# dbolya/yolact

Measured on AMD Instinct MI355X. Metric: images/sec (550x550, batch 8 per GPU), YOLACT yolact_resnet50 forward + Detect (Fast NMS), higher is better.
Workload: dtype f32 (fp32 in / fp32 accumulate / fp32 out; 93 % of the GEMM time on fp16x2 tiles = every fp32 operand as two fp16 pieces by round to nearest (22 significant bits + 2 signs: exact for ~2/3 of all fp32 values, one fp32 ulp otherwise), 3 exact piece products per product on the fp16 matrix pipe; measure

## Files before the change

include/yolact_amd.h:

```cpp
#ifndef YOLACT_AMD_H
#define YOLACT_AMD_H
#include <stddef.h>
#include <stdint.h>

#ifdef __cplusplus
extern "C" {
#endif

#define YMI_ABI_VERSION 9

#define YMI_EFORMAT (-4)
#define YMI_EUNSUPPORTED (-5)

enum { YMI_ACT_NONE = 0, YMI_ACT_RELU = 1, YMI_ACT_LEAKY01 = 2, YMI_ACT_TANH = 3, YMI_ACT_SIGMOID = 4 };
enum { YMI_RES_NONE = 0, YMI_RES_ADD = 1, YMI_RES_BILINEAR = 2 };

typedef struct {
  int32_t n0, n1;
  int32_t act;
  int32_t row_stride;
  int64_t batch_stride;
  float *ptr;
} ymi_conv_seg;

// ... 217 lines not shown
  int32_t out_width, out_height;
  int32_t hs[3], vs[3];
  int32_t hf[3], vf[3];
  int32_t bw[3], bh[3];
  int32_t dw[3], dh[3];
  int64_t coef_count;
  int64_t plane_bytes;
} ymi_jpeg_info;
int ymi_jpeg_parse(const uint8_t *data, size_t n, ymi_jpeg_info *info);
int ymi_jpeg_decode_coefs(const uint8_t *data, size_t n, int16_t *coefs, int64_t coef_capacity, uint16_t *qt,
                          ymi_jpeg_info *info);
int ymi_jpeg_reconstruct_bgr_u8(const ymi_jpeg_info *info, const int16_t *coefs, const uint16_t *qt, uint8_t *planes_ws,
                                uint8_t *out, void *stream);

int ymi_coco_poly_fill_u8(const double *xy, int k, int h, int w, uint8_t *mask);
int ymi_coco_rle_fill_u8(const uint32_t *counts, long n, int h, int w, uint8_t *mask);
int ymi_coco_rle_string_fill_u8(const char *s, long len, int h, int w, uint8_t *mask);

typedef struct {
  ymi_conv_desc conv;
  const float *offmask;
  int32_t ldo;
  int32_t mask_is_prob;
  int32_t om_layout;
  int32_t _pad1;
} ymi_dcn_desc;
int ymi_dcn_v2_forward_f32(const ymi_dcn_desc *d, void *stream);

typedef struct ymi_stem_desc {
  const float *x;
  float *y;
  int32_t B, H, W, cout_pad;
  const void *w_h2;
  const float *scale_h2, *bias;
  float *y_amax;
  int32_t kpad, _pad0;
} ymi_stem_desc;
int ymi_stem_pool_f32(const ymi_stem_desc *d, void *stream);

typedef struct ymi_chain_desc {
  const float *x, *res;
  float *y, *z;
  const void *w_a_h2, *w_b_h2;
  const float *scale_a_h2, *bias_a, *scale_b_h2, *bias_b;
  const float *x_amax;
  float *y_amax, *z_amax;
  int64_t M;
  int32_t ldx, res_ld, ldy, ldz;
  int32_t k_a, n_a, n_b;
  int32_t cout_pad_a, cout_pad_b;
  int32_t act_a, act_b, _pad0;
  const float *res_amax;
  float gain_a, bias_max_a;
} ymi_chain_desc;
int ymi_pointwise_chain_f32(const ymi_chain_desc *d, void *stream);

enum { YMI_OP_NOP = 0, YMI_OP_CONV = 1, YMI_OP_WINO = 2, YMI_OP_DCN = 3, YMI_OP_CHAIN = 4, YMI_OP_STEM = 5, YMI_OP_INPUT = 6,
       YMI_OP_BILINEAR = 7, YMI_OP_MAXPOOL = 8, YMI_OP_BILINEAR_ADD = 9, YMI_OP_RECORD = 10, YMI_OP_WAIT = 11, YMI_OP_MEMSET = 12 };
enum { YMI_SEC_NONE = 0, YMI_SEC_BACKBONE = 1, YMI_SEC_FPN = 2, YMI_SEC_PROTO = 3, YMI_SEC_HEADS = 4 };
typedef struct ymi_plan_op {
  int32_t kind;
  int32_t stream;
  int32_t section;
  int32_t _pad;
  const void *desc;
  void *p[3];
  int64_t i[8];
  double f[2];
} ymi_plan_op;
int ymi_event_create(void **ev);
int ymi_event_destroy(void *ev);
int ymi_plan_run(const ymi_plan_op *ops, int first, int last, void *stream_a, void *stream_b, void *const *events, int overlap,
                 int skip_sections, int32_t *failed_op);

enum {
  YMI_WS_WINO_V = 1,
  YMI_WS_WINO_M = 2,
  YMI_WS_SPLITK = 3,
  YMI_WS_MASK_IOU = 4,
  YMI_WS_JPEG_COEFS = 5,
  YMI_WS_JPEG_PLANES = 6,
  YMI_WS_DETECT_SCORES_T = 7,
  YMI_WS_DETECT_PER_PRIOR = 8,
  YMI_WS_DETECT_CAND = 9,
  YMI_WS_DETECT_REC = 10,
  YMI_WS_AMAX_SLOT = 11,
  YMI_WS_RLE_COUNTS = 12,
  YMI_WS_DETECT_GREEDY = 13
};
typedef struct { int32_t A, B; int64_t n; } ymi_mask_iou_shape;
typedef struct { int32_t N, h, w, cap; } ymi_rle_shape;
int64_t ymi_workspace_bytes(int what, const void *desc);

int ymi_calib_mfma_f16(float *out, int blocks, int iters, double *flops, void *stream);
int ymi_calib_hbm_copy(const float *src, float *dst, long n_floats, double *bytes, void *stream);
int ymi_calib_l2_read(const float *src, long n_floats, int blocks, int iters, float *out, double *bytes, void *stream);
int ymi_calib_latency(const int32_t *chain, long n, int start, int hops, int32_t *out, void *stream);

int ymi_debug_set_trace(void *buf, long cap_blocks);
int ymi_prof_enable(int on);
int ymi_prof_count(void);
int ymi_prof_read(int i, float *ms, double *flops, int32_t *tile, int32_t *kind);
int ymi_prof_reset(void);

#ifdef __cplusplus
}
// ... 3 lines not shown
```

yolact_amd/_lib.py:

```python
from __future__ import annotations

import ctypes as C
import os

_HERE = os.path.dirname(os.path.abspath(__file__))
LIB_PATH = os.path.join(_HERE, 'libyolact_amd.so')

ABI_VERSION = 9

ACT_NONE, ACT_RELU, ACT_LEAKY01, ACT_TANH, ACT_SIGMOID = 0, 1, 2, 3, 4
RES_NONE, RES_ADD, RES_BILINEAR = 0, 1, 2
TILE_AUTO, TILE_128x128, TILE_128x64, TILE_64x64, TILE_128x32, TILE_64x128 = 0, 1, 2, 3, 4, 5
TILE_32x32_K4, TILE_64x32_K2, TILE_32x64_K2 = 6, 7, 8
TILE_64x64_S3, TILE_64x64_S4, TILE_64x128_S3, TILE_128x64_S3, TILE_32x32_K4_S4, TILE_64x32_K2_S3, TILE_32x64_K2_S3 = range(9, 16)
TILE_NAMES = {1: '128x128', 2: '128x64', 3: '64x64', 4: '128x32', 5: '64x128', 6: '32x32k4', 7: '64x32k2', 8: '32x64k2',
              9: '64x64s3', 10: '64x64s4', 11: '64x128s3', 12: '128x64s3', 13: '32x32k4s4', 14: '64x32k2s3', 15: '32x64k2s3',
              16: '128x128w8', 17: '256x128w8', 18: '128x256w8', 19: '128x128s3', 20: '128x128w8s3', 21: '256x128w8s3',
              22: '128x128w8s4'}
TILE_128x128_W8, TILE_256x128_W8, TILE_128x256_W8 = 16, 17, 18
TILE_128x128_S3, TILE_128x128_W8_S3, TILE_256x128_W8_S3, TILE_128x128_W8_S4 = 19, 20, 21, 22
TILE_WG_128x256 = 23
TILE_X3 = 32
X3_BASE_TILES = (1, 2, 3, 5, 6, 7, 8, 9, 11, 12, 16, 17, 19, 20, 21, 22)
for _t in X3_BASE_TILES:
# ... 50 lines not shown


class WinoDesc(C.Structure):
    _fields_ = [('x', C.c_void_p), ('u', C.c_void_p), ('scale', C.c_void_p), ('bias', C.c_void_p), ('y', C.c_void_p),
                ('V', C.c_void_p), ('M', C.c_void_p),
                ('B', C.c_int32), ('H', C.c_int32), ('W', C.c_int32), ('C', C.c_int32), ('Cout', C.c_int32),
                ('act', C.c_int32), ('tile', C.c_int32), ('nseg', C.c_int32), ('m', C.c_int32), ('_pad0', C.c_int32),
                ('seg', ConvSeg * 3), ('u_x3', C.c_void_p), ('cout_alg', C.c_int32), ('v_planes', C.c_int32),
                ('u_h2', C.c_void_p), ('uinv_h2', C.c_void_p), ('x_amax', C.c_void_p), ('y_amax', C.c_void_p),
                ('x_up', C.c_void_p), ('up_relu', C.c_int32), ('_pad4', C.c_int32),
                ('proj_w_h2', C.c_void_p), ('proj_scale_h2', C.c_void_p), ('proj_bias', C.c_void_p),
                ('proj_y', C.c_void_p), ('proj_y_amax', C.c_void_p),
                ('proj_cout', C.c_int32), ('proj_ldy', C.c_int32), ('proj_act', C.c_int32), ('_pad5', C.c_int32)]


class DcnDesc(C.Structure):
    _fields_ = [('conv', ConvDesc), ('offmask', C.c_void_p), ('ldo', C.c_int32), ('mask_is_prob', C.c_int32),
                ('om_layout', C.c_int32), ('_pad1', C.c_int32)]


class DetectDesc(C.Structure):
    _fields_ = [('conf', C.c_void_p), ('loc', C.c_void_p), ('coef', C.c_void_p), ('priors', C.c_void_p),
                ('B', C.c_int32), ('P', C.c_int32), ('C', C.c_int32), ('D', C.c_int32),
                ('conf_is_logits', C.c_int32), ('top_k', C.c_int32), ('max_det', C.c_int32),
                ('conf_thresh', C.c_float), ('nms_thresh', C.c_float), ('cross_class', C.c_int32),
                ('conf_ld', C.c_int32), ('_pad1', C.c_int32),
                ('scores_t', C.c_void_p), ('keep', C.c_void_p), ('num_keep', C.c_void_p),
                ('maxsc', C.c_void_p), ('argmax', C.c_void_p),
                ('cand_score', C.c_void_p), ('cand_prior', C.c_void_p),
                ('out_count', C.c_void_p), ('out_box', C.c_void_p), ('out_score', C.c_void_p),
                ('out_class', C.c_void_p), ('out_coef', C.c_void_p), ('out_prior', C.c_void_p), ('out_rec', C.c_void_p)]


class DetectGreedyWs(C.Structure):
    _fields_ = [('box_scale', C.c_float), ('_pad0', C.c_int32), ('ws', C.c_void_p)]


class JpegInfo(C.Structure):
    _fields_ = [('width', C.c_int32), ('height', C.c_int32), ('ncomp', C.c_int32), ('progressive', C.c_int32),
                ('orientation', C.c_int32), ('color', C.c_int32), ('out_width', C.c_int32), ('out_height', C.c_int32),
                ('hs', C.c_int32 * 3), ('vs', C.c_int32 * 3), ('hf', C.c_int32 * 3), ('vf', C.c_int32 * 3),
                ('bw', C.c_int32 * 3), ('bh', C.c_int32 * 3), ('dw', C.c_int32 * 3), ('dh', C.c_int32 * 3),
                ('coef_count', C.c_int64), ('plane_bytes', C.c_int64)]


class ChainDesc(C.Structure):
    _fields_ = [('x', C.c_void_p), ('res', C.c_void_p), ('y', C.c_void_p), ('z', C.c_void_p),
                ('w_a_h2', C.c_void_p), ('w_b_h2', C.c_void_p),
                ('scale_a_h2', C.c_void_p), ('bias_a', C.c_void_p), ('scale_b_h2', C.c_void_p), ('bias_b', C.c_void_p),
                ('x_amax', C.c_void_p), ('y_amax', C.c_void_p), ('z_amax', C.c_void_p),
                ('M', C.c_int64), ('ldx', C.c_int32), ('res_ld', C.c_int32), ('ldy', C.c_int32), ('ldz', C.c_int32),
                ('k_a', C.c_int32), ('n_a', C.c_int32), ('n_b', C.c_int32), ('cout_pad_a', C.c_int32), ('cout_pad_b', C.c_int32),
                ('act_a', C.c_int32), ('act_b', C.c_int32), ('_pad0', C.c_int32),
                ('res_amax', C.c_void_p), ('gain_a', C.c_float), ('bias_max_a', C.c_float)]


class StemDesc(C.Structure):
    _fields_ = [('x', C.c_void_p), ('y', C.c_void_p), ('B', C.c_int32), ('H', C.c_int32), ('W', C.c_int32), ('cout_pad', C.c_int32),
                ('w_h2', C.c_void_p), ('scale_h2', C.c_void_p), ('bias', C.c_void_p), ('y_amax', C.c_void_p),
                ('kpad', C.c_int32), ('_pad0', C.c_int32)]


class PlanOp(C.Structure):
    _fields_ = [('kind', C.c_int32), ('stream', C.c_int32), ('section', C.c_int32), ('_pad', C.c_int32), ('desc', C.c_void_p),
                ('p', C.c_void_p * 3), ('i', C.c_int64 * 8), ('f', C.c_double * 2)]


(OP_NOP, OP_CONV, OP_WINO, OP_DCN, OP_CHAIN, OP_STEM, OP_INPUT, OP_BILINEAR, OP_MAXPOOL, OP_BILINEAR_ADD, OP_RECORD, OP_WAIT,
 OP_MEMSET) = range(13)
SEC_NONE, SEC_BACKBONE, SEC_FPN, SEC_PROTO, SEC_HEADS = range(5)


class MaskIouShape(C.Structure):
    _fields_ = [('A', C.c_int32), ('B', C.c_int32), ('n', C.c_int64)]


class ApMatchDesc(C.Structure):
    _fields_ = [('cls', C.c_void_p), ('box_score', C.c_void_p), ('mask_score', C.c_void_p), ('box_iou', C.c_void_p),
                ('mask_iou', C.c_void_p), ('crowd_box_iou', C.c_void_p), ('crowd_mask_iou', C.c_void_p), ('gt_cls', C.c_void_p),
                ('crowd_cls', C.c_void_p), ('rec_key', C.c_void_p), ('rec_score', C.c_void_p), ('rec_flags', C.c_void_p),
                ('gt_count', C.c_void_p), ('base', C.c_int64), ('cap', C.c_int64),
                ('N', C.c_int32), ('G', C.c_int32), ('Gc', C.c_int32), ('num_classes', C.c_int32)]


class ApFinalizeDesc(C.Structure):
    _fields_ = [('sorted_key', C.c_void_p), ('perm', C.c_void_p), ('rec_flags', C.c_void_p), ('gt_count', C.c_void_p),
                ('ap', C.c_void_p), ('empty', C.c_void_p), ('M', C.c_int64), ('cap', C.c_int64),
                ('num_classes', C.c_int32), ('_pad0', C.c_int32)]


AP_NUM_THRESH, AP_MAX_DET, AP_MAX_GT = 10, 1024, 2048


class RleShape(C.Structure):
    _fields_ = [('N', C.c_int32), ('h', C.c_int32), ('w', C.c_int32), ('cap', C.c_int32)]


(WS_WINO_V, WS_WINO_M, WS_SPLITK, WS_MASK_IOU, WS_JPEG_COEFS, WS_JPEG_PLANES, WS_DETECT_SCORES_T, WS_DETECT_PER_PRIOR,
 WS_DETECT_CAND, WS_DETECT_REC, WS_AMAX_SLOT, WS_RLE_COUNTS, WS_DETECT_GREEDY) = range(1, 14)

EFORMAT, EUNSUPPORTED = -4, -5

_P, _I, _F = C.c_void_p, C.c_int, C.c_float
SYMBOLS = [
    ('ymi_abi_version', C.c_int, []),
    ('ymi_strerror', C.c_char_p, [C.c_int]),
    ('ymi_conv2d_nhwc_f32', C.c_int, [C.POINTER(ConvDesc), _P]),
# ... 93 lines not shown
```

yolact_amd/csrc/chain.hip:

```cpp
#include "common.h"
#include <type_traits>
#include "../../include/yolact_amd.h"

int ymi_internal_prof_begin(double flops, int tile, int kind, hipStream_t s);
void ymi_internal_prof_end(int idx, hipStream_t s);

namespace {

typedef _Float16 f16x8 __attribute__((ext_vector_type(8)));
typedef _Float16 f16x4 __attribute__((ext_vector_type(4)));
typedef unsigned u32x4 __attribute__((ext_vector_type(4)));

constexpr int K1 = 64, N1 = 256, N2 = 64, PX = 32, NW = 8;
constexpr int RS1 = 2 * K1 + 16;
constexpr int RS2 = 2 * N1 + 16;
constexpr int A1_PLANE = PX * RS1, A2_PLANE = PX * RS2;
constexpr int A1_BUF = 2 * A1_PLANE, A2_BUF = 2 * A2_PLANE;
constexpr int OFF_A1 = 0, OFF_A2 = OFF_A1 + 2 * A1_BUF, OFF_SC = OFF_A2 + 2 * A2_BUF, OFF_EP = OFF_SC + 2 * (2 * NW * 4),
              CH_LDS = OFF_EP + NW * 2 * 4 * 32;

struct ChainParams {
  const float *x, *res, *x_amax;
  const void *wa, *wb;
  const float *sa, *ba, *sb, *bb;
  float *y, *z, *y_amax, *z_amax;
  int M, ldx, res_ld, ldy, ldz, act_a, act_b;
  unsigned wa_plane, wb_plane;
};

__global__ __launch_bounds__(64 * NW) void chain_h2_k(const ChainParams p) {
#if defined(__HIP_DEVICE_COMPILE__)
  __shared__ __attribute__((aligned(16))) char lds[CH_LDS];
  const int t = threadIdx.x, lane = t & 63, wave = __builtin_amdgcn_readfirstlane(t >> 6);
  const int lr = lane & 15, g = lane >> 4;
  const int q2 = wave & 3, i2 = wave >> 2;
  float sA, invA;
  ymi_h2_scale(ymi_amax_read(p.x_amax), sA, invA);
  const ymi_amax_pre apre_y = ymi_amax_prefetch(p.y_amax);
  const ymi_amax_pre apre_z = ymi_amax_prefetch(p.z_amax);
  const bool two = p.z != nullptr;

  f16x8 w3h[2][2], w3l[2][2], w1h[8], w1l[8];
#pragma unroll
  for (int j = 0; j < 2; ++j)
#pragma unroll
    for (int c = 0; c < 2; ++c) {
      const char *src = reinterpret_cast<const char *>(p.wa) + (size_t)(32 * wave + 16 * j + lr) * (2 * K1) + c * 64 + g * 16;
      w3h[j][c] = *reinterpret_cast<const f16x8 *>(src);
      w3l[j][c] = *reinterpret_cast<const f16x8 *>(src + p.wa_plane);
    }
#pragma unroll
  for (int c = 0; c < 8; ++c) {
    const f16x8 z8 = {0, 0, 0, 0, 0, 0, 0, 0};
    const char *src = reinterpret_cast<const char *>(p.wb) + (size_t)(16 * q2 + lr) * (2 * N1) + c * 64 + g * 16;
    w1h[c] = two ? *reinterpret_cast<const f16x8 *>(src) : z8;
    w1l[c] = two ? *reinterpret_cast<const f16x8 *>(src + p.wb_plane) : z8;
  }
  if (lr == 0) {
#pragma unroll
    for (int j = 0; j < 2; ++j) {
      const int n = 32 * wave + 16 * j + 4 * g;
      f32x4 sc, bi;
#pragma unroll
      for (int e = 0; e < 4; ++e) { sc[e] = p.sa[n + e] * invA; bi[e] = p.ba ? p.ba[n + e] : 0.f; }
      *reinterpret_cast<f32x4 *>(lds + OFF_EP + ((wave * 2 + j) * 4 + g) * 32) = sc;
      *reinterpret_cast<f32x4 *>(lds + OFF_EP + ((wave * 2 + j) * 4 + g) * 32 + 16) = bi;
    }
  }
  f32x4 sc1 = {1.f, 1.f, 1.f, 1.f}, bi1 = {0.f, 0.f, 0.f, 0.f};
  if (two) {
#pragma unroll
    for (int e = 0; e < 4; ++e) { sc1[e] = p.sb[16 * q2 + 4 * g + e]; bi1[e] = p.bb ? p.bb[16 * q2 + 4 * g + e] : 0.f; }
  }
  const float slope_a = p.act_a == YMI_ACT_RELU ? 0.f : (p.act_a == YMI_ACT_LEAKY01 ? 0.1f : 1.f);
  const float slope_b = p.act_b == YMI_ACT_RELU ? 0.f : (p.act_b == YMI_ACT_LEAKY01 ? 0.1f : 1.f);

  const int ntiles = (p.M + PX - 1) / PX;
  constexpr unsigned OOB = 0x80000000u;
  const __amdgpu_buffer_rsrc_t xrs = __builtin_amdgcn_make_buffer_rsrc((void *)p.x, 0, (int)((unsigned)p.M * (unsigned)p.ldx * 4u), 0x00020000);
  const __amdgpu_buffer_rsrc_t rrs = __builtin_amdgcn_make_buffer_rsrc((void *)(p.res ? p.res : p.x), 0, p.res ? (int)((unsigned)p.M * (unsigned)p.res_ld * 4u) : 0, 0x00020000);
  const __amdgpu_buffer_rsrc_t yrs = __builtin_amdgcn_make_buffer_rsrc((void *)p.y, 0, (int)((unsigned)p.M * (unsigned)p.ldy * 4u), 0x00020000);
  const __amdgpu_buffer_rsrc_t zrs = __builtin_amdgcn_make_buffer_rsrc((void *)(p.z ? p.z : p.y), 0, p.z ? (int)((unsigned)p.M * (unsigned)p.ldz * 4u) : 0, 0x00020000);
  const int xp = t >> 4, xc = t & 15;
  auto load_x = [&](int tile) {
    const int m = tile * PX + xp;
    const unsigned off = (tile < ntiles && m < p.M) ? (unsigned)(m * p.ldx + 4 * xc) * 4u : OOB;
    return __builtin_bit_cast(f32x4, __builtin_amdgcn_raw_buffer_load_b128(xrs, off, 0, 0));
  };
  auto load_res = [&](int tile, f32x4 (&r)[2][2]) {
#pragma unroll
    for (int i = 0; i < 2; ++i) {
      const int m = tile * PX + 16 * i + lr;
      const unsigned off = (tile < ntiles && m < p.M) ? (unsigned)(m * p.res_ld + 32 * wave + 4 * g) * 4u : OOB;
#pragma unroll
      for (int j = 0; j < 2; ++j) r[i][j] = __builtin_bit_cast(f32x4, __builtin_amdgcn_raw_buffer_load_b128(rrs, off + 64u * j, 0, 0));
    }
  };

#define CHAIN_BARRIER() asm volatile("s_waitcnt lgkmcnt(0)\n\ts_barrier" ::: "memory")
  float am_y = 0.f, am_z = 0.f;
  f32x4 xv;
  const int grid = (int)gridDim.x;
  auto iteration = [&](const int tile, auto buf_c, f32x4 (&rv)[2][2], f32x4 (&rn)[2][2]) {
    constexpr int BUF = decltype(buf_c)::value;
    char *const a1 = lds + OFF_A1 + BUF * A1_BUF;
    char *const a2w = lds + OFF_A2 + BUF * A2_BUF;
    const char *const a2r = lds + OFF_A2 + (BUF ^ 1) * A2_BUF;
    float *const scw = reinterpret_cast<float *>(lds + OFF_SC) + BUF * (2 * NW);
    const float *const scr = reinterpret_cast<const float *>(lds + OFF_SC) + (BUF ^ 1) * (2 * NW);
    {
      const f32x4 v = xv * sA;
      f16x4 h4, l4;
#pragma unroll
      for (int e = 0; e < 4; ++e) {
        const _Float16 h = (_Float16)v[e];
        h4[e] = h;
        l4[e] = (_Float16)(v[e] - (float)h);
      }
      char *dst = a1 + xp * RS1 + xc * 8;
      *reinterpret_cast<f16x4 *>(dst) = h4;
      *reinterpret_cast<f16x4 *>(dst + A1_PLANE) = l4;
    }
    xv = load_x(tile + grid);
    load_res(tile + grid, rn);
    CHAIN_BARRIER();
    if (two) {
      f32x4 tot = {0.f, 0.f, 0.f, 0.f};
#pragma unroll
      for (int c0 = 0; c0 < 8; c0 += 2) {
        f16x8 xh[2], xl[2];
        f32x4 a2[2];
#pragma unroll
        for (int u = 0; u < 2; ++u) {
          xh[u] = *reinterpret_cast<const f16x8 *>(a2r + (16 * i2 + lr) * RS2 + (c0 + u) * 64 + g * 16);
          xl[u] = *reinterpret_cast<const f16x8 *>(a2r + A2_PLANE + (16 * i2 + lr) * RS2 + (c0 + u) * 64 + g * 16);
          a2[u] = f32x4{0.f, 0.f, 0.f, 0.f};
        }
#pragma unroll
        for (int pr = 0; pr < 3; ++pr)
#pragma unroll
          for (int u = 0; u < 2; ++u)
            a2[u] = ymi_mfma16(pr == 0 ? w1l[c0 + u] : w1h[c0 + u], pr == 1 ? xl[u] : xh[u], a2[u]);
#pragma unroll
        for (int u = 0; u < 2; ++u) tot += a2[u] * scr[i2 * NW + c0 + u];
      }
      const int tp = tile - grid, m = tp * PX + 16 * i2 + lr;
      const bool ok = tp >= 0 && m < p.M;
      f32x4 v = tot * sc1 + bi1;
#pragma unroll
      for (int e = 0; e < 4; ++e) v[e] = fmaxf(v[e], slope_b * v[e]);
      am_z = fmaxf(am_z, ok ? ymi_absmax4(v) : 0.f);
      __builtin_amdgcn_raw_buffer_store_b128(__builtin_bit_cast(u32x4, v), zrs, ok ? (unsigned)(m * p.ldz + 16 * q2 + 4 * g) * 4u : OOB, 0, 0);
    }
    f32x4 acc[2][2];
#pragma unroll
    for (int i = 0; i < 2; ++i)
#pragma unroll
      for (int j = 0; j < 2; ++j) acc[i][j] = f32x4{0.f, 0.f, 0.f, 0.f};
#pragma unroll
    for (int c = 0; c < 2; ++c) {
      f16x8 xh[2], xl[2];
#pragma unroll
      for (int i = 0; i < 2; ++i) {
        xh[i] = *reinterpret_cast<const f16x8 *>(a1 + (16 * i + lr) * RS1 + c * 64 + g * 16);
        xl[i] = *reinterpret_cast<const f16x8 *>(a1 + A1_PLANE + (16 * i + lr) * RS1 + c * 64 + g * 16);
      }
#pragma unroll
      for (int pr = 0; pr < 3; ++pr)
#pragma unroll
        for (int i = 0; i < 2; ++i)
#pragma unroll
          for (int j = 0; j < 2; ++j)
            acc[i][j] = ymi_mfma16(pr == 0 ? w3l[j][c] : w3h[j][c], pr == 1 ? xl[i] : xh[i], acc[i][j]);
    }
#pragma unroll
    for (int i = 0; i < 2; ++i) {
      const int m = tile * PX + 16 * i + lr;
      const bool ok = m < p.M;
      const unsigned yoff = ok ? (unsigned)(m * p.ldy + 32 * wave + 4 * g) * 4u : OOB;
      float tm = 0.f;
#pragma unroll
      for (int j = 0; j < 2; ++j) {
        const f32x4 sc3 = *reinterpret_cast<const f32x4 *>(lds + OFF_EP + ((wave * 2 + j) * 4 + g) * 32);
        const f32x4 bi3 = *reinterpret_cast<const f32x4 *>(lds + OFF_EP + ((wave * 2 + j) * 4 + g) * 32 + 16);
        f32x4 v = acc[i][j] * sc3 + bi3 + rv[i][j];
#pragma unroll
        for (int e = 0; e < 4; ++e) v[e] = fmaxf(v[e], slope_a * v[e]);
        if (!ok) v = f32x4{0.f, 0.f, 0.f, 0.f};
        acc[i][j] = v;
        tm = fmaxf(tm, ymi_absmax4(v));
        __builtin_amdgcn_raw_buffer_store_b128(__builtin_bit_cast(u32x4, v), yrs, yoff + 64u * j, 0, 0);
      }
      am_y = fmaxf(am_y, tm);
      if (two) {
        const unsigned tmb = ymi_wave_umax63(__builtin_bit_cast(unsigned, tm));
        float sT, invT;
        ymi_h2_scale(__builtin_bit_cast(float, (unsigned)__builtin_amdgcn_readlane((int)tmb, 63)), sT, invT);
#pragma unroll
        for (int j = 0; j < 2; ++j) {
          const f32x4 v = acc[i][j] * sT;
          f16x4 h4, l4;
#pragma unroll
          for (int e = 0; e < 4; ++e) {
            const _Float16 h = (_Float16)v[e];
            h4[e] = h;
            l4[e] = (_Float16)(v[e] - (float)h);
          }
          char *dst = a2w + (16 * i + lr) * RS2 + (32 * wave + 16 * j + 4 * g) * 2;
          *reinterpret_cast<f16x4 *>(dst) = h4;
          *reinterpret_cast<f16x4 *>(dst + A2_PLANE) = l4;
        }
        if (lane == 0) scw[i * NW + wave] = invT;
      }
    }
  };
  int tile = blockIdx.x;
  f32x4 ra[2][2], rb[2][2];
  xv = load_x(tile);
  load_res(tile, ra);
  for (; tile < ntiles + (two ? grid : 0); tile += 2 * grid) {
    iteration(tile, std::integral_constant<int, 0>{}, ra, rb);
    iteration(tile + grid, std::integral_constant<int, 1>{}, rb, ra);
  }
#undef CHAIN_BARRIER
  if (p.y_amax) ymi_amax_finish(apre_y, am_y);
  if (two && p.z_amax) ymi_amax_finish(apre_z, am_z);
#endif
}

}

int ymi_internal_chain2(const ymi_chain_desc *d, hipStream_t s);

extern "C" int ymi_pointwise_chain_f32(const ymi_chain_desc *d, void *stream) {
  if (!d) return YMI_ENULL;
  if (!d->x || !d->w_a_h2 || !d->scale_a_h2 || !d->y || !d->x_amax) return YMI_ENULL;
  if (d->z && (!d->w_b_h2 || !d->scale_b_h2)) return YMI_ENULL;
  const bool wide = d->k_a == 128 || d->k_a == 256;
  if (d->M <= 0 || (!wide && (d->k_a != K1 || d->n_a != N1 || (d->z && d->n_b != N2)))) return YMI_EARG;
  if (wide && (d->n_a != 4 * d->k_a || (d->z && d->n_b != d->k_a))) return YMI_EARG;
  if (d->act_a < 0 || d->act_a > YMI_ACT_LEAKY01 || d->act_b < 0 || d->act_b > YMI_ACT_LEAKY01) return YMI_EARG;
  if (d->ldx < d->k_a || d->ldy < d->n_a || (d->z && d->ldz < d->n_b) || (d->res && d->res_ld < d->n_a)) return YMI_ESHAPE;
  if ((d->ldx | d->ldy | d->ldz | d->res_ld) & 3) return YMI_ESHAPE;
  if ((((uintptr_t)d->x) | ((uintptr_t)d->y) | ((uintptr_t)d->z) | ((uintptr_t)d->res) | ((uintptr_t)d->w_a_h2) | ((uintptr_t)d->w_b_h2)) & 15)
    return YMI_ESHAPE;
  if (d->M * (int64_t)(d->ldy > d->res_ld ? d->ldy : d->res_ld) >= (1LL << 29) || d->M * (int64_t)d->ldx >= (1LL << 29)) return YMI_ESHAPE;
  if (wide) return ymi_internal_chain2(d, (hipStream_t)stream);
  if (d->cout_pad_a < N1 || (d->z && d->cout_pad_b < N2)) return YMI_ESHAPE;
  ChainParams p;
  p.x = d->x; p.res = d->res; p.x_amax = d->x_amax; p.wa = d->w_a_h2; p.wb = d->w_b_h2;
  p.sa = d->scale_a_h2; p.ba = d->bias_a; p.sb = d->scale_b_h2; p.bb = d->bias_b;
  p.y = d->y; p.z = d->z; p.y_amax = d->y_amax; p.z_amax = d->z_amax;
  p.M = (int)d->M; p.ldx = d->ldx; p.res_ld = d->res_ld; p.ldy = d->ldy; p.ldz = d->ldz; p.act_a = d->act_a; p.act_b = d->act_b;
  p.wa_plane = (unsigned)((long)d->cout_pad_a * K1 * 2); p.wb_plane = (unsigned)((long)d->cout_pad_b * N1 * 2);
  hipStream_t s = (hipStream_t)stream;
  const int pr = ymi_internal_prof_begin(2.0 * (double)d->M * K1 * N1, YMI_TILE_H2 | YMI_TILE_64x64, 13, s);
  int dev = 0, cus = 256;
  hipGetDevice(&dev);
  hipDeviceGetAttribute(&cus, hipDeviceAttributeMultiprocessorCount, dev);
  const long ntiles = (d->M + PX - 1) / PX;
  hipLaunchKernelGGL(chain_h2_k, dim3((unsigned)(ntiles < cus ? ntiles : cus)), dim3(64 * NW), 0, s, p);
  const int rc = ymi_launch_status();
  ymi_internal_prof_end(pr, s);
  if (rc == YMI_OK && d->z) {
    const int p2 = ymi_internal_prof_begin(2.0 * (double)d->M * N1 * N2, YMI_TILE_H2 | YMI_TILE_64x64, 12, s);
    ymi_internal_prof_end(p2, s);
  }
  return rc;
}
```

yolact_amd/engine.py:

```python
from __future__ import annotations

import ctypes as C
import json
import os
from typing import List, Optional

import torch
import torch.nn as nn

from . import _lib as L
from .config import act_name, make_priors_host
from . import modules as M


def _ceil(a, b):
    return (a + b - 1) // b * b


SPLIT_DEFAULT = '2'
TUNE_GEN = 5
AMAX_SLOT_FLOATS = 16 * 64
TUNE_DIR = os.path.join(os.path.dirname(os.path.abspath(__file__)), 'tune')
_table_cache = {}

# ... 1191 lines not shown
                rc = fn(*args, s)
            else:
                rc = fn(args, s)
            if rc != 0:
                L.check(rc, name)
        return det

    def tune(self, x: torch.Tensor, reps: int = 3):
        mode = os.environ.get('YOLACT_AMD_AUTOTUNE', '1')
        self.tune_table, self.wino_table, self.tune_misses = [], [], 0
        if mode == '0':
            return []
        cache_path = os.environ.get('YOLACT_AMD_TUNE_CACHE')
        disk = {}
        if mode != 'force':
            disk.update(load_tune_table(self.device))
            if cache_path and os.path.exists(cache_path):
                disk.update(_read_table_file(cache_path))
        n0 = len(disk)
        self.run(x)
        s = L.stream_ptr()
        e0, e1 = torch.cuda.Event(enable_timing=True), torch.cuda.Event(enable_timing=True)
        measure = mode != 'table'
        self._tune_direct(e0, e1, s, reps, disk, measure)
        self._tune_winograd(e0, e1, s, reps, disk, measure)
        self._fuse_pointwise_chains(e0, e1, s, reps, disk, measure)
        torch.cuda.synchronize(self.device)
        if cache_path and (len(disk) != n0 or mode == 'force'):
            _write_table_file(cache_path, disk, self.device)
        self.tune_entries = disk
        return self.tune_table

    autotune = tune

    def _splitk_ws(self, where, numel):
        ws = self._sk_ws.get(where)
        if ws is None or ws.numel() < numel:
            ws = self._sk_ws[where] = torch.empty(numel, dtype=torch.float32, device=self.device)
            for fn, dptr, _n, w in self.ops:
                if fn is self.lib.ymi_conv2d_nhwc_f32 and w == where and dptr.contents.split_k > 1:
                    dptr.contents.split_ws = ws.data_ptr()
                elif fn is self.lib.ymi_dcn_v2_forward_f32 and w == where and dptr.contents.conv.split_k > 1:
                    dptr.contents.conv.split_ws = ws.data_ptr()
        return ws

    @staticmethod
    def _splitk_ok(d):
        return (d.kh == 1 and d.kw == 1 and d.pad == 0 and d.Cin == d.Kpad and d.Cin % 32 == 0 and d.nseg == 1
                and d.Cout % 4 == 0 and d.seg[0].act <= L.ACT_LEAKY01 and d.res_mode in (L.RES_NONE, L.RES_ADD)
                and d.B * d.Ho * d.Wo <= 16384 and d.Kpad >= 256)

    def _fuse_pointwise_chains(self, e0, e1, s, reps, disk, measure):
        self.chain_table = []
        if not self.h2 or os.environ.get('YOLACT_AMD_CHAIN', '1') != '1':
            return
        lib = self.lib

        def timed(run):
            run()
            best = 1e30
            for _ in range(2):
                e0.record()
                for _ in range(reps):
                    run()
                e1.record()
                e1.synchronize()
                best = min(best, e0.elapsed_time(e1) / reps)
            return best
        i = 0
        while i < len(self.ops):
            f3, p3, n3, w3 = self.ops[i]
            i += 1
            if f3 is not lib.ymi_conv2d_nhwc_f32 or (i - 1) in self.wide_ops:
                continue
            d3 = p3.contents
            M = d3.B * d3.Ho * d3.Wo
            P_ = d3.Cin
            if not ((d3.kh, d3.kw, d3.stride, d3.pad, d3.nseg) == (1, 1, 1, 0, 1) and P_ in (64, 128, 256) and d3.Cout == 4 * P_
                    and d3.res_mode == L.RES_ADD and not d3.res_after_act and d3.seg[0].n0 == 0 and d3.seg[0].act <= L.ACT_LEAKY01
                    and d3.w_h2 and d3.x_amax and M * max(d3.seg[0].row_stride, d3.res_ld) < (1 << 29)):
                continue
            if P_ > 64 and os.environ.get('YOLACT_AMD_CHAIN2', '0') not in ('1', 'force'):
                continue
            pair = False
            if i < len(self.ops) and self.ops[i][0] is lib.ymi_conv2d_nhwc_f32 and self.ops[i][3] == w3 and i not in self.wide_ops:
                d1 = self.ops[i][1].contents
                pair = ((d1.kh, d1.kw, d1.stride, d1.pad, d1.Cin, d1.Cout, d1.nseg) == (1, 1, 1, 0, 4 * P_, P_, 1)
                        and d1.res_mode == L.RES_NONE and d1.x == d3.seg[0].ptr and d1.ldx == d3.seg[0].row_stride
                        and d1.seg[0].n0 == 0 and d1.seg[0].act <= L.ACT_LEAKY01 and bool(d1.w_h2))
            if P_ > 64 and not pair:
                continue
            cd = L.ChainDesc()
            cd.x, cd.res, cd.y = d3.x, d3.res, d3.seg[0].ptr
            cd.w_a_h2, cd.scale_a_h2, cd.bias_a = d3.w_h2, d3.scale_h2, d3.bias
            cd.x_amax, cd.y_amax = d3.x_amax, d3.y_amax
            cd.M, cd.ldx, cd.res_ld, cd.ldy = M, d3.ldx, d3.res_ld, d3.seg[0].row_stride
            cd.k_a, cd.n_a, cd.n_b, cd.cout_pad_a, cd.cout_pad_b = P_, 4 * P_, P_, _ceil(4 * P_, 128), _ceil(P_, 128)
            cd.act_a = d3.seg[0].act
            if P_ > 64:
                info = getattr(self, '_desc_info', {}).get(C.addressof(d3))
                if info is None or info[1] is None:
                    continue
                cd.gain_a, cd.bias_max_a = info[0].l1_gain()
                cd.res_amax = self._slot_ptr(info[1])
            name = n3
            if pair:
                f1, p1, n1, w1 = self.ops[i]
                cd.z, cd.ldz, cd.z_amax, cd.act_b = d1.seg[0].ptr, d1.seg[0].row_stride, d1.y_amax, d1.seg[0].act
                cd.w_b_h2, cd.scale_b_h2, cd.bias_b = d1.w_h2, d1.scale_h2, d1.bias
                name = n3 + '+' + n1
            if pair:
                def span(ptr, ld):
                    return (int(ptr), int(ptr) + 4 * M * int(ld))

                def overlap(a, b):
                    return a[0] < b[1] and b[0] < a[1]
                zs, xs = span(cd.z, cd.ldz), span(cd.x, cd.ldx)
                in_place = int(cd.z) == int(cd.x) and cd.ldz == cd.ldx
                if overlap(zs, span(cd.y, cd.ldy)) or overlap(zs, span(cd.res, cd.res_ld)) or (overlap(zs, xs) and not in_place):
                    continue
            cptr = C.pointer(cd)
            key = ('chain' if pair else 'chain1') + str((d3.B, d3.Ho, d3.Wo) + ((P_,) if P_ > 64 else ())) + self.mode_key
            ent = disk.get(key)
            if P_ > 64 and os.environ.get('YOLACT_AMD_CHAIN2') == 'force':
                ent = [1, 0.0, 0.0]
            if ent is None:
                self.tune_misses += 1
                if not measure or lib.ymi_pointwise_chain_f32(cptr, s) != 0:
                    continue
                t_plan = timed((lambda: (f3(p3, s), f1(p1, s))) if pair else (lambda: f3(p3, s)))
                t_one = timed(lambda: lib.ymi_pointwise_chain_f32(cptr, s))
                ent = disk[key] = [1 if t_one < 0.97 * t_plan else 0, round(t_plan, 4), round(t_one, 4)]
            self.chain_table.append((name, ent[0], ent[1], ent[2]))
            if ent[0] and lib.ymi_pointwise_chain_f32(cptr, s) == 0:
                self.keepalive.append(cd)
                self.ops[i - 1] = (lib.ymi_pointwise_chain_f32, cptr, name, w3)
                if pair:
                    self.ops[i] = ('nop', None, n1 + '[fused into ' + n3 + ']', w1)
                    i += 1

    def _apply_choice(self, fn, dptr, where, val, s):
        d = dptr.contents.conv if fn is self.lib.ymi_dcn_v2_forward_f32 else dptr.contents
        tile, S = int(val) & 255, int(val) >> 8
        d.tile = tile
        if S > 1:
            is_dcn = fn is self.lib.ymi_dcn_v2_forward_f32
            if tile & L.TILE_DCNP:
                nk_ = d.Kpad // 32
                if -(-nk_ // S) * (S - 1) >= nk_:
                    return -1
            elif is_dcn or not self._splitk_ok(d) or (d.Kpad // 32) % S:
                return -1
            d.split_k = S
            d.split_ws = self._splitk_ws(where, S * d.B * d.Ho * d.Wo * d.Cout).data_ptr()
        else:
            d.split_k = 0
        return fn(dptr, s)

    @staticmethod
    def _pipe_ok(d):
        return ((d.kh, d.kw, d.pad) in ((3, 3, 1), (1, 1, 0)) and d.Cin % 32 == 0 and d.Kpad == d.kh * d.kw * d.Cin and d.Kpad >= 64
                and d.nseg == 1 and d.Cout % 4 == 0 and d.seg[0].n0 == 0 and d.seg[0].act <= L.ACT_LEAKY01
                and d.seg[0].row_stride % 4 == 0 and d.seg[0].batch_stride == d.Ho * d.Wo * d.seg[0].row_stride
                and d.res_mode in (L.RES_NONE, L.RES_ADD))

    @staticmethod
    def dcnp_candidates(d, dcn=False):
        M, nk = d.B * d.Ho * d.Wo, d.Kpad // 32
        out = []
        for t, name in sorted(L.DCNP_TILES.items()):
            bm, bn = (int(v) for v in name[4:].split('w')[0].split('x'))
            if (bn > 128 and d.Cout < 256) or (dcn and t in L.DCNP_PLAIN_ONLY) or (bn == 32) != (d.Cout <= 32):
                continue
            tid = t | L.TILE_H2 | L.TILE_DCNP
            out.append(tid)
            blocks = -(-M // bm) * -(-d.Cout // bn)
            if blocks < 400 and d.Cout % 4 == 0:
                for S in (2, 3, 4, 5, 6, 8, 9, 12, 16):
                    per = -(-nk // S)
                    if per >= 4 and per * (S - 1) < nk and 128 <= blocks * S <= 1100:
                        out.append(tid + 256 * S)
        return out

    @staticmethod
    def patch2_candidates(d):
        if os.environ.get('YOLACT_AMD_PATCH2', '1') != '1':
# ... 270 lines not shown
```

Measured before the change: 2333.

## Fuse bottleneck downsample projection conv into pointwise chain kernel

Adds a PROJ variant of the chain kernel that computes the 1x1 downsample projection (64->256) of the block input alongside the expanding 1x1 conv. The projection result serves as the residual directly, so it is never written to and read back from global memory. The engine finds the matching '.down' conv, checks aliasing, autotunes fused against unfused, and replaces the down op with a nop. This costs extra LDS, registers and MFMA work per tile, which may lower occupancy, and it affects only the first block of the P=64 stage.

```diff
diff --git a/include/yolact_amd.h b/include/yolact_amd.h
--- a/include/yolact_amd.h
+++ b/include/yolact_amd.h
@@ -293,6 +293,10 @@
   int32_t act_a, act_b, _pad0;
   const float *res_amax;
   float gain_a, bias_max_a;
+  const float *x2, *x2_amax;
+  const void *w_p_h2;
+  const float *scale_p_h2, *bias_p;
+  int32_t ldx2, cout_pad_p;
 } ymi_chain_desc;
 int ymi_pointwise_chain_f32(const ymi_chain_desc *d, void *stream);
 
diff --git a/yolact_amd/_lib.py b/yolact_amd/_lib.py
--- a/yolact_amd/_lib.py
+++ b/yolact_amd/_lib.py
@@ -126,7 +126,9 @@
                 ('M', C.c_int64), ('ldx', C.c_int32), ('res_ld', C.c_int32), ('ldy', C.c_int32), ('ldz', C.c_int32),
                 ('k_a', C.c_int32), ('n_a', C.c_int32), ('n_b', C.c_int32), ('cout_pad_a', C.c_int32), ('cout_pad_b', C.c_int32),
                 ('act_a', C.c_int32), ('act_b', C.c_int32), ('_pad0', C.c_int32),
-                ('res_amax', C.c_void_p), ('gain_a', C.c_float), ('bias_max_a', C.c_float)]
+                ('res_amax', C.c_void_p), ('gain_a', C.c_float), ('bias_max_a', C.c_float),
+                ('x2', C.c_void_p), ('x2_amax', C.c_void_p), ('w_p_h2', C.c_void_p), ('scale_p_h2', C.c_void_p),
+                ('bias_p', C.c_void_p), ('ldx2', C.c_int32), ('cout_pad_p', C.c_int32)]
 
 
 class StemDesc(C.Structure):
diff --git a/yolact_amd/csrc/chain.hip b/yolact_amd/csrc/chain.hip
--- a/yolact_amd/csrc/chain.hip
+++ b/yolact_amd/csrc/chain.hip
@@ -18,6 +18,7 @@
 constexpr int A1_BUF = 2 * A1_PLANE, A2_BUF = 2 * A2_PLANE;
 constexpr int OFF_A1 = 0, OFF_A2 = OFF_A1 + 2 * A1_BUF, OFF_SC = OFF_A2 + 2 * A2_BUF, OFF_EP = OFF_SC + 2 * (2 * NW * 4),
               CH_LDS = OFF_EP + NW * 2 * 4 * 32;
+constexpr int OFF_AP = CH_LDS, OFF_EPP = OFF_AP + 2 * A1_BUF, CH_LDS_PROJ = OFF_EPP + NW * 2 * 4 * 32;
 
 struct ChainParams {
   const float *x, *res, *x_amax;
@@ -26,21 +27,29 @@
   float *y, *z, *y_amax, *z_amax;
   int M, ldx, res_ld, ldy, ldz, act_a, act_b;
   unsigned wa_plane, wb_plane;
+  const float *x2, *x2_amax, *sp, *bp;
+  const void *wp;
+  int ldx2;
+  unsigned wp_plane;
 };
 
+template <bool PROJ>
 __global__ __launch_bounds__(64 * NW) void chain_h2_k(const ChainParams p) {
 #if defined(__HIP_DEVICE_COMPILE__)
-  __shared__ __attribute__((aligned(16))) char lds[CH_LDS];
+  __shared__ __attribute__((aligned(16))) char lds[PROJ ? CH_LDS_PROJ : CH_LDS];
   const int t = threadIdx.x, lane = t & 63, wave = __builtin_amdgcn_readfirstlane(t >> 6);
   const int lr = lane & 15, g = lane >> 4;
   const int q2 = wave & 3, i2 = wave >> 2;
   float sA, invA;
   ymi_h2_scale(ymi_amax_read(p.x_amax), sA, invA);
+  float sX = 1.f, invX = 1.f;
+  if constexpr (PROJ) ymi_h2_scale(ymi_amax_read(p.x2_amax), sX, invX);
   const ymi_amax_pre apre_y = ymi_amax_prefetch(p.y_amax);
   const ymi_amax_pre apre_z = ymi_amax_prefetch(p.z_amax);
   const bool two = p.z != nullptr;
 
   f16x8 w3h[2][2], w3l[2][2], w1h[8], w1l[8];
+  f16x8 wph[PROJ ? 2 : 1][2], wpl[PROJ ? 2 : 1][2];
 #pragma unroll
   for (int j = 0; j < 2; ++j)
 #pragma unroll
@@ -48,6 +57,11 @@
       const char *src = reinterpret_cast<const char *>(p.wa) + (size_t)(32 * wave + 16 * j + lr) * (2 * K1) + c * 64 + g * 16;
       w3h[j][c] = *reinterpret_cast<const f16x8 *>(src);
       w3l[j][c] = *reinterpret_cast<const f16x8 *>(src + p.wa_plane);
+      if constexpr (PROJ) {
+        const char *sp_ = reinterpret_cast<const char *>(p.wp) + (size_t)(32 * wave + 16 * j + lr) * (2 * K1) + c * 64 + g * 16;
+        wph[j][c] = *reinterpret_cast<const f16x8 *>(sp_);
+        wpl[j][c] = *reinterpret_cast<const f16x8 *>(sp_ + p.wp_plane);
+      }
     }
 #pragma unroll
   for (int c = 0; c < 8; ++c) {
@@ -65,6 +79,12 @@
       for (int e = 0; e < 4; ++e) { sc[e] = p.sa[n + e] * invA; bi[e] = p.ba ? p.ba[n + e] : 0.f; }
       *reinterpret_cast<f32x4 *>(lds + OFF_EP + ((wave * 2 + j) * 4 + g) * 32) = sc;
       *reinterpret_cast<f32x4 *>(lds + OFF_EP + ((wave * 2 + j) * 4 + g) * 32 + 16) = bi;
+      if constexpr (PROJ) {
+#pragma unroll
+        for (int e = 0; e < 4; ++e) { sc[e] = p.sp[n + e] * invX; bi[e] = p.bp ? p.bp[n + e] : 0.f; }
+        *reinterpret_cast<f32x4 *>(lds + OFF_EPP + ((wave * 2 + j) * 4 + g) * 32) = sc;
+        *reinterpret_cast<f32x4 *>(lds + OFF_EPP + ((wave * 2 + j) * 4 + g) * 32 + 16) = bi;
+      }
     }
   }
   f32x4 sc1 = {1.f, 1.f, 1.f, 1.f}, bi1 = {0.f, 0.f, 0.f, 0.f};
@@ -81,7 +101,13 @@
   const __amdgpu_buffer_rsrc_t rrs = __builtin_amdgcn_make_buffer_rsrc((void *)(p.res ? p.res : p.x), 0, p.res ? (int)((unsigned)p.M * (unsigned)p.res_ld * 4u) : 0, 0x00020000);
   const __amdgpu_buffer_rsrc_t yrs = __builtin_amdgcn_make_buffer_rsrc((void *)p.y, 0, (int)((unsigned)p.M * (unsigned)p.ldy * 4u), 0x00020000);
   const __amdgpu_buffer_rsrc_t zrs = __builtin_amdgcn_make_buffer_rsrc((void *)(p.z ? p.z : p.y), 0, p.z ? (int)((unsigned)p.M * (unsigned)p.ldz * 4u) : 0, 0x00020000);
+  const __amdgpu_buffer_rsrc_t x2rs = __builtin_amdgcn_make_buffer_rsrc((void *)(PROJ ? p.x2 : p.x), 0, PROJ ? (int)((unsigned)p.M * (unsigned)p.ldx2 * 4u) : 0, 0x00020000);
   const int xp = t >> 4, xc = t & 15;
+  auto load_x2 = [&](int tile) {
+    const int m = tile * PX + xp;
+    const unsigned off = (tile < ntiles && m < p.M) ? (unsigned)(m * p.ldx2 + 4 * xc) * 4u : OOB;
+    return __builtin_bit_cast(f32x4, __builtin_amdgcn_raw_buffer_load_b128(x2rs, off, 0, 0));
+  };
   auto load_x = [&](int tile) {
     const int m = tile * PX + xp;
     const unsigned off = (tile < ntiles && m < p.M) ? (unsigned)(m * p.ldx + 4 * xc) * 4u : OOB;
@@ -99,7 +125,7 @@
 
 #define CHAIN_BARRIER() asm volatile("s_waitcnt lgkmcnt(0)\n\ts_barrier" ::: "memory")
   float am_y = 0.f, am_z = 0.f;
-  f32x4 xv;
+  f32x4 xv, x2v;
   const int grid = (int)gridDim.x;
   auto iteration = [&](const int tile, auto buf_c, f32x4 (&rv)[2][2], f32x4 (&rn)[2][2]) {
     constexpr int BUF = decltype(buf_c)::value;
@@ -121,8 +147,23 @@
       *reinterpret_cast<f16x4 *>(dst) = h4;
       *reinterpret_cast<f16x4 *>(dst + A1_PLANE) = l4;
     }
+    char *const ap = lds + OFF_AP + BUF * A1_BUF;
+    if constexpr (PROJ) {
+      const f32x4 v = x2v * sX;
+      f16x4 h4, l4;
+#pragma unroll
+      for (int e = 0; e < 4; ++e) {
+        const _Float16 h = (_Float16)v[e];
+        h4[e] = h;
+        l4[e] = (_Float16)(v[e] - (float)h);
+      }
+      char *dst = ap + xp * RS1 + xc * 8;
+      *reinterpret_cast<f16x4 *>(dst) = h4;
+      *reinterpret_cast<f16x4 *>(dst + A1_PLANE) = l4;
+    }
     xv = load_x(tile + grid);
-    load_res(tile + grid, rn);
+    if constexpr (PROJ) x2v = load_x2(tile + grid);
+    else load_res(tile + grid, rn);
     CHAIN_BARRIER();
     if (two) {
       f32x4 tot = {0.f, 0.f, 0.f, 0.f};
@@ -153,25 +194,27 @@
       __builtin_amdgcn_raw_buffer_store_b128(__builtin_bit_cast(u32x4, v), zrs, ok ? (unsigned)(m * p.ldz + 16 * q2 + 4 * g) * 4u : OOB, 0, 0);
     }
     f32x4 acc[2][2];
-#pragma unroll
-    for (int i = 0; i < 2; ++i)
-#pragma unroll
-      for (int j = 0; j < 2; ++j) acc[i][j] = f32x4{0.f, 0.f, 0.f, 0.f};
-#pragma unroll
-    for (int c = 0; c < 2; ++c) {
-      f16x8 xh[2], xl[2];
-#pragma unroll
-      for (int i = 0; i < 2; ++i) {
-        xh[i] = *reinterpret_cast<const f16x8 *>(a1 + (16 * i + lr) * RS1 + c * 64 + g * 16);
-        xl[i] = *reinterpret_cast<const f16x8 *>(a1 + A1_PLANE + (16 * i + lr) * RS1 + c * 64 + g * 16);
-      }
-#pragma unroll
-      for (int pr = 0; pr < 3; ++pr)
-#pragma unroll
-        for (int i = 0; i < 2; ++i)
-#pragma unroll
-          for (int j = 0; j < 2; ++j)
-            acc[i][j] = ymi_mfma16(pr == 0 ? w3l[j][c] : w3h[j][c], pr == 1 ? xl[i] : xh[i], acc[i][j]);
+    if constexpr (!PROJ) {
+#pragma unroll
+      for (int i = 0; i < 2; ++i)
+#pragma unroll
+        for (int j = 0; j < 2; ++j) acc[i][j] = f32x4{0.f, 0.f, 0.f, 0.f};
+#pragma unroll
+      for (int c = 0; c < 2; ++c) {
+        f16x8 xh[2], xl[2];
+#pragma unroll
+        for (int i = 0; i < 2; ++i) {
+          xh[i] = *reinterpret_cast<const f16x8 *>(a1 + (16 * i + lr) * RS1 + c * 64 + g * 16);
+          xl[i] = *reinterpret_cast<const f16x8 *>(a1 + A1_PLANE + (16 * i + lr) * RS1 + c * 64 + g * 16);
+        }
+#pragma unroll
+        for (int pr = 0; pr < 3; ++pr)
+#pragma unroll
+          for (int i = 0; i < 2; ++i)
+#pragma unroll
+            for (int j = 0; j < 2; ++j)
+              acc[i][j] = ymi_mfma16(pr == 0 ? w3l[j][c] : w3h[j][c], pr == 1 ? xl[i] : xh[i], acc[i][j]);
+      }
     }
 #pragma unroll
     for (int i = 0; i < 2; ++i) {
@@ -179,11 +222,37 @@
       const bool ok = m < p.M;
       const unsigned yoff = ok ? (unsigned)(m * p.ldy + 32 * wave + 4 * g) * 4u : OOB;
       float tm = 0.f;
+      f32x4 accp[2];
+      if constexpr (PROJ) {
+#pragma unroll
+        for (int j = 0; j < 2; ++j) { acc[i][j] = f32x4{0.f, 0.f, 0.f, 0.f}; accp[j] = f32x4{0.f, 0.f, 0.f, 0.f}; }
+#pragma unroll
+        for (int c = 0; c < 2; ++c) {
+          const int fo = (16 * i + lr) * RS1 + c * 64 + g * 16;
+          const f16x8 xh = *reinterpret_cast<const f16x8 *>(a1 + fo), xl = *reinterpret_cast<const f16x8 *>(a1 + A1_PLANE + fo);
+          const f16x8 qh = *reinterpret_cast<const f16x8 *>(ap + fo), ql = *reinterpret_cast<const f16x8 *>(ap + A1_PLANE + fo);
+#pragma unroll
+          for (int pr = 0; pr < 3; ++pr)
+#pragma unroll
+            for (int j = 0; j < 2; ++j) {
+              acc[i][j] = ymi_mfma16(pr == 0 ? w3l[j][c] : w3h[j][c], pr == 1 ? xl : xh, acc[i][j]);
+              accp[j] = ymi_mfma16(pr == 0 ? wpl[j][c] : wph[j][c], pr == 1 ? ql : qh, accp[j]);
+            }
+        }
+      }
 #pragma unroll
       for (int j = 0; j < 2; ++j) {
         const f32x4 sc3 = *reinterpret_cast<const f32x4 *>(lds + OFF_EP + ((wave * 2 + j) * 4 + g) * 32);
         const f32x4 bi3 = *reinterpret_cast<const f32x4 *>(lds + OFF_EP + ((wave * 2 + j) * 4 + g) * 32 + 16);
-        f32x4 v = acc[i][j] * sc3 + bi3 + rv[i][j];
+        f32x4 rsd;
+        if constexpr (PROJ) {
+          const f32x4 scp = *reinterpret_cast<const f32x4 *>(lds + OFF_EPP + ((wave * 2 + j) * 4 + g) * 32);
+          const f32x4 bip = *reinterpret_cast<const f32x4 *>(lds + OFF_EPP + ((wave * 2 + j) * 4 + g) * 32 + 16);
+          rsd = accp[j] * scp + bip;
+        } else {
+          rsd = rv[i][j];
+        }
+        f32x4 v = acc[i][j] * sc3 + bi3 + rsd;
 #pragma unroll
         for (int e = 0; e < 4; ++e) v[e] = fmaxf(v[e], slope_a * v[e]);
         if (!ok) v = f32x4{0.f, 0.f, 0.f, 0.f};
@@ -217,7 +286,8 @@
   int tile = blockIdx.x;
   f32x4 ra[2][2], rb[2][2];
   xv = load_x(tile);
-  load_res(tile, ra);
+  if constexpr (PROJ) x2v = load_x2(tile);
+  else load_res(tile, ra);
   for (; tile < ntiles + (two ? grid : 0); tile += 2 * grid) {
     iteration(tile, std::integral_constant<int, 0>{}, ra, rb);
     iteration(tile + grid, std::integral_constant<int, 1>{}, rb, ra);
@@ -247,21 +317,35 @@
   if (d->M * (int64_t)(d->ldy > d->res_ld ? d->ldy : d->res_ld) >= (1LL << 29) || d->M * (int64_t)d->ldx >= (1LL << 29)) return YMI_ESHAPE;
   if (wide) return ymi_internal_chain2(d, (hipStream_t)stream);
   if (d->cout_pad_a < N1 || (d->z && d->cout_pad_b < N2)) return YMI_ESHAPE;
+  const bool proj = !d->res && d->x2;
+  if (proj) {
+    if (!d->x2_amax || !d->w_p_h2 || !d->scale_p_h2) return YMI_ENULL;
+    if (d->ldx2 < K1 || (d->ldx2 & 3) || d->cout_pad_p < N1) return YMI_ESHAPE;
+    if ((((uintptr_t)d->x2) | ((uintptr_t)d->w_p_h2)) & 15) return YMI_ESHAPE;
+    if (d->M * (int64_t)d->ldx2 >= (1LL << 29)) return YMI_ESHAPE;
+  }
   ChainParams p;
   p.x = d->x; p.res = d->res; p.x_amax = d->x_amax; p.wa = d->w_a_h2; p.wb = d->w_b_h2;
   p.sa = d->scale_a_h2; p.ba = d->bias_a; p.sb = d->scale_b_h2; p.bb = d->bias_b;
   p.y = d->y; p.z = d->z; p.y_amax = d->y_amax; p.z_amax = d->z_amax;
   p.M = (int)d->M; p.ldx = d->ldx; p.res_ld = d->res_ld; p.ldy = d->ldy; p.ldz = d->ldz; p.act_a = d->act_a; p.act_b = d->act_b;
   p.wa_plane = (unsigned)((long)d->cout_pad_a * K1 * 2); p.wb_plane = (unsigned)((long)d->cout_pad_b * N1 * 2);
+  p.x2 = proj ? d->x2 : nullptr; p.x2_amax = d->x2_amax; p.wp = d->w_p_h2; p.sp = d->scale_p_h2; p.bp = d->bias_p;
+  p.ldx2 = d->ldx2; p.wp_plane = proj ? (unsigned)((long)d->cout_pad_p * K1 * 2) : 0u;
   hipStream_t s = (hipStream_t)stream;
   const int pr = ymi_internal_prof_begin(2.0 * (double)d->M * K1 * N1, YMI_TILE_H2 | YMI_TILE_64x64, 13, s);
   int dev = 0, cus = 256;
   hipGetDevice(&dev);
   hipDeviceGetAttribute(&cus, hipDeviceAttributeMultiprocessorCount, dev);
   const long ntiles = (d->M + PX - 1) / PX;
-  hipLaunchKernelGGL(chain_h2_k, dim3((unsigned)(ntiles < cus ? ntiles : cus)), dim3(64 * NW), 0, s, p);
+  if (proj) hipLaunchKernelGGL(chain_h2_k<true>, dim3((unsigned)(ntiles < cus ? ntiles : cus)), dim3(64 * NW), 0, s, p);
+  else hipLaunchKernelGGL(chain_h2_k<false>, dim3((unsigned)(ntiles < cus ? ntiles : cus)), dim3(64 * NW), 0, s, p);
   const int rc = ymi_launch_status();
   ymi_internal_prof_end(pr, s);
+  if (rc == YMI_OK && proj) {
+    const int p1 = ymi_internal_prof_begin(2.0 * (double)d->M * K1 * N1, YMI_TILE_H2 | YMI_TILE_64x64, 12, s);
+    ymi_internal_prof_end(p1, s);
+  }
   if (rc == YMI_OK && d->z) {
     const int p2 = ymi_internal_prof_begin(2.0 * (double)d->M * N1 * N2, YMI_TILE_H2 | YMI_TILE_64x64, 12, s);
     ymi_internal_prof_end(p2, s);
diff --git a/yolact_amd/engine.py b/yolact_amd/engine.py
--- a/yolact_amd/engine.py
+++ b/yolact_amd/engine.py
@@ -1267,6 +1267,7 @@
 
     def _fuse_pointwise_chains(self, e0, e1, s, reps, disk, measure):
         self.chain_table = []
+        self.proj_table = []
         if not self.h2 or os.environ.get('YOLACT_AMD_CHAIN', '1') != '1':
             return
         lib = self.lib
@@ -1319,6 +1320,18 @@
                 cd.gain_a, cd.bias_max_a = info[0].l1_gain()
                 cd.res_amax = self._slot_ptr(info[1])
             name = n3
+            down_i, proj_mode = None, os.environ.get('YOLACT_AMD_PROJ', '1')
+            if P_ == 64 and proj_mode != '0':
+                for k in range(i - 2, -1, -1):
+                    fk, pk_, nk_, _wk = self.ops[k]
+                    if fk is lib.ymi_conv2d_nhwc_f32 and pk_.contents.nseg == 1 and pk_.contents.seg[0].ptr == d3.res:
+                        dd = pk_.contents
+                        if (nk_.endswith('.down') and (dd.kh, dd.kw, dd.stride, dd.pad, dd.Cin, dd.Cout) == (1, 1, 1, 0, 64, 256)
+                                and dd.res_mode == L.RES_NONE and dd.seg[0].n0 == 0 and dd.seg[0].act == L.ACT_NONE
+                                and dd.seg[0].row_stride == d3.res_ld and dd.B * dd.Ho * dd.Wo == M and dd.w_h2 and dd.x_amax
+                                and dd.ldx % 4 == 0 and k not in self.wide_ops and M * dd.ldx < (1 << 29)):
+                            down_i = k
+                        break
             if pair:
                 f1, p1, n1, w1 = self.ops[i]
                 cd.z, cd.ldz, cd.z_amax, cd.act_b = d1.seg[0].ptr, d1.seg[0].row_stride, d1.y_amax, d1.seg[0].act
@@ -1334,6 +1347,10 @@
                 in_place = int(cd.z) == int(cd.x) and cd.ldz == cd.ldx
                 if overlap(zs, span(cd.y, cd.ldy)) or overlap(zs, span(cd.res, cd.res_ld)) or (overlap(zs, xs) and not in_place):
                     continue
+                if down_i is not None:
+                    dd = self.ops[down_i][1].contents
+                    if overlap(zs, span(dd.x, dd.ldx)) and not (int(cd.z) == int(dd.x) and cd.ldz == dd.ldx):
+                        down_i = None
             cptr = C.pointer(cd)
             key = ('chain' if pair else 'chain1') + str((d3.B, d3.Ho, d3.Wo) + ((P_,) if P_ > 64 else ())) + self.mode_key
             ent = disk.get(key)
@@ -1347,6 +1364,34 @@
                 t_one = timed(lambda: lib.ymi_pointwise_chain_f32(cptr, s))
                 ent = disk[key] = [1 if t_one < 0.97 * t_plan else 0, round(t_plan, 4), round(t_one, 4)]
             self.chain_table.append((name, ent[0], ent[1], ent[2]))
+            if ent[0] and down_i is not None:
+                fd, pd, nd, wd = self.ops[down_i]
+                dd = pd.contents
+                cp = L.ChainDesc()
+                C.memmove(C.addressof(cp), C.addressof(cd), C.sizeof(cd))
+                cp.res, cp.res_ld = None, 0
+                cp.x2, cp.ldx2, cp.x2_amax = dd.x, dd.ldx, dd.x_amax
+                cp.w_p_h2, cp.scale_p_h2, cp.bias_p, cp.cout_pad_p = dd.w_h2, dd.scale_h2, dd.bias, _ceil(256, 128)
+                pptr = C.pointer(cp)
+                pkey = 'proj' + str((d3.B, d3.Ho, d3.Wo, 64, 64, 256, 1)) + self.mode_key
+                pent = disk.get(pkey)
+                if proj_mode == 'force':
+                    pent = [1, 0.0, 0.0, 0]
+                if pent is None:
+                    self.tune_misses += 1
+                    if measure and lib.ymi_pointwise_chain_f32(pptr, s) == 0:
+                        t_two = timed(lambda: (fd(pd, s), lib.ymi_pointwise_chain_f32(cptr, s)))
+                        t_fused = timed(lambda: lib.ymi_pointwise_chain_f32(pptr, s))
+                        pent = disk[pkey] = [1 if t_fused < 0.97 * t_two else 0, round(t_two, 4), round(t_fused, 4), 0]
+                if pent is not None:
+                    self.proj_table.append((nd, pent[0], pent[1], pent[2]))
+                    if pent[0] and lib.ymi_pointwise_chain_f32(pptr, s) == 0:
+                        cd, cptr = cp, pptr
+                        self.ops[down_i] = ('nop', None, nd + '[fused into ' + n3 + ']', wd)
+                        mi = [k for k, (n_, _d) in enumerate(self.conv_meta) if n_ == nd]
+                        m3 = [k for k, (n_, _d) in enumerate(self.conv_meta) if n_ == n3]
+                        if len(mi) == 1 and len(m3) == 1 and mi[0] < m3[0]:
+                            self.conv_meta.insert(m3[0], self.conv_meta.pop(mi[0]))
             if ent[0] and lib.ymi_pointwise_chain_f32(cptr, s) == 0:
                 self.keepalive.append(cd)
                 self.ops[i - 1] = (lib.ymi_pointwise_chain_f32, cptr, name, w3)
```

Measured after the change: 2364 (median of 6 runs). 1.3% higher.
